# mdw771/beyond_dof

Hardware: AMD Instinct MI355X
Metric: multislice fwd+adjoint slice-steps/s (full Adam iteration: rotation, forward, loss, adjoint, gradient exchange, regulariser+Adam) (higher is better)
Workload: dtype f32

## Files before the change

### beyond_dof_amd/csrc/bdof_fft.h

```cpp
#pragma once
#include <hip/hip_runtime.h>

typedef float2 cf;

__device__ __forceinline__ cf cadd(cf a, cf b) { return make_float2(a.x + b.x, a.y + b.y); }
__device__ __forceinline__ cf csub(cf a, cf b) { return make_float2(a.x - b.x, a.y - b.y); }
__device__ __forceinline__ cf cmul(cf a, cf b) { return make_float2(a.x * b.x - a.y * b.y, a.x * b.y + a.y * b.x); }
__device__ __forceinline__ cf cmulc(cf a, cf b) { return make_float2(a.x * b.x + a.y * b.y, a.y * b.x - a.x * b.y); }
__device__ __forceinline__ cf cscale(cf a, float s) { return make_float2(a.x * s, a.y * s); }


template <int SIGN, bool EX> __device__ __forceinline__ cf tw_mul(cf u, cf w, cf wl) {
    if (SIGN > 0) { w.y = -w.y; wl.y = -wl.y; }
    if constexpr (EX) {
        const float lx = fmaf(u.x, wl.x, -(u.y * wl.y)), ly = fmaf(u.x, wl.y, u.y * wl.x);
        return make_float2(fmaf(u.x, w.x, fmaf(-u.y, w.y, lx)), fmaf(u.x, w.y, fmaf(u.y, w.x, ly)));
    } else return cmul(u, w);
}

template <int SIGN> __device__ __forceinline__ cf mul_si(cf a) {
    return SIGN > 0 ? make_float2(-a.y, a.x) : make_float2(a.y, -a.x);
}

template <int SIGN> __device__ __forceinline__ void dft2(cf& a, cf& b) {
    cf t = a;
    a = cadd(t, b);
    b = csub(t, b);
}

template <int SIGN> __device__ __forceinline__ void dft4(cf& a0, cf& a1, cf& a2, cf& a3) {
    cf s0 = cadd(a0, a2), s1 = csub(a0, a2), s2 = cadd(a1, a3), s3 = mul_si<SIGN>(csub(a1, a3));
    a0 = cadd(s0, s2);
    a2 = csub(s0, s2);
    a1 = cadd(s1, s3);
    a3 = csub(s1, s3);
}

template <int ROUND_> __device__ __forceinline__ float mul_sqrt_half(float t, const float* sq = nullptr) {
    if constexpr (ROUND_ != 0) {
        if (sq) return t * sq[ROUND_ - 1];
    }
    return fmaf(t, 0.70710678118654752f, t * 1.2101617e-8f);
}

template <int SIGN, int ROUND = 1>
__device__ __forceinline__ void dft8(cf& a0, cf& a1, cf& a2, cf& a3, cf& a4, cf& a5, cf& a6, cf& a7, const float* sq = nullptr) {
    dft4<SIGN>(a0, a2, a4, a6);
    dft4<SIGN>(a1, a3, a5, a7);
    const float s = (float)SIGN;
    cf o0 = a1;
    cf o1 = make_float2(mul_sqrt_half<ROUND>(a3.x - s * a3.y, sq), mul_sqrt_half<ROUND>(a3.y + s * a3.x, sq));
    cf o2 = mul_si<SIGN>(a5);
    cf o3 = make_float2(mul_sqrt_half<ROUND>(-a7.x - s * a7.y, sq), mul_sqrt_half<ROUND>(-a7.y + s * a7.x, sq));
    cf e0 = a0, e1 = a2, e2 = a4, e3 = a6;
    a0 = cadd(e0, o0); a4 = csub(e0, o0);
    a1 = cadd(e1, o1); a5 = csub(e1, o1);
    a2 = cadd(e2, o2); a6 = csub(e2, o2);
    a3 = cadd(e3, o3); a7 = csub(e3, o3);
}

template <int N> struct FftPlan;
template <> struct FftPlan<64>   { static constexpr int NS = 2, R0 = 8, R1 = 8, R2 = 1, R3 = 1; };
template <> struct FftPlan<128>  { static constexpr int NS = 3, R0 = 8, R1 = 2, R2 = 8, R3 = 1; };
template <> struct FftPlan<256>  { static constexpr int NS = 3, R0 = 8, R1 = 4, R2 = 8, R3 = 1; };
template <> struct FftPlan<512>  { static constexpr int NS = 3, R0 = 8, R1 = 8, R2 = 8, R3 = 1; };
template <> struct FftPlan<1024> { static constexpr int NS = 4, R0 = 8, R1 = 2, R2 = 8, R3 = 8; };

template <int N> struct FftTw {
    typedef FftPlan<N> P;
    static constexpr int RL = P::NS == 2 ? P::R1 : (P::NS == 3 ? P::R2 : P::R3);
    static constexpr int PL = N / RL;
    static constexpr int M1_R = P::NS > 2 ? P::R1 : 1, M1_P = P::R0;
    static constexpr int M2_R = P::NS > 3 ? P::R2 : 1, M2_P = P::R0 * P::R1;
    static constexpr int M1_OFF = 0, M1_CNT = P::NS > 2 ? M1_P * (M1_R - 1) : 0;
    static constexpr int M2_OFF = M1_CNT, M2_CNT = P::NS > 3 ? M2_P * (M2_R - 1) : 0;
    static constexpr int LDS_CNT = M1_CNT + M2_CNT > 0 ? M1_CNT + M2_CNT : 1;
    static constexpr int D1 = M1_R > 1 ? M1_R - 1 : 1, D2 = M2_R > 1 ? M2_R - 1 : 1;
    cf w[7];
    const cf* mid;
    const cf* tail;
    const float* sq = nullptr;

    template <bool LO = false>
    __device__ __forceinline__ void load(const cf* __restrict__ table, int tid, cf* lds_mid, cf* lds_tail) {
        constexpr int T = N / 8;
        for (int e = threadIdx.x; e < 7 * T; e += blockDim.x) {
            const int m = e / T + 1, j = e - (m - 1) * T;
            lds_tail[e] = table[m * j];
            if constexpr (LO) lds_tail[7 * T + e] = table[N + m * j];
        }
        for (int e = threadIdx.x; e < M1_CNT + M2_CNT; e += blockDim.x) {
            int k, m, step;
            if (e < M1_CNT) { k = e / D1; m = e % D1 + 1; step = N / (M1_P * M1_R); }
            else { const int f = e - M1_CNT; k = f / D2; m = f % D2 + 1; step = N / (M2_P * M2_R); }
            lds_mid[e] = table[m * k * step];
            if constexpr (LO) lds_mid[LDS_CNT + e] = table[N + m * k * step];
        }
        mid = lds_mid;
        tail = lds_tail;
        __syncthreads();
#pragma unroll
        for (int m = 1; m < 8; ++m) w[m - 1] = lds_tail[(m - 1) * T + tid];
    }
};

template <int R, int SIGN, int ROUND = 1> __device__ __forceinline__ void dftR(cf (&u)[8], int j, const float* sq = nullptr) {
    if constexpr (R == 8) dft8<SIGN, ROUND>(u[0], u[1], u[2], u[3], u[4], u[5], u[6], u[7], sq);
    else if constexpr (R == 4) {
        if (j == 0) dft4<SIGN>(u[0], u[1], u[2], u[3]); else dft4<SIGN>(u[4], u[5], u[6], u[7]);
    } else {
        if (j == 0) dft2<SIGN>(u[0], u[1]); else if (j == 1) dft2<SIGN>(u[2], u[3]);
        else if (j == 2) dft2<SIGN>(u[4], u[5]); else dft2<SIGN>(u[6], u[7]);
    }
}

template <int N, int R, class L> __device__ __forceinline__ void stage_read(cf (&u)[8], int tid, L& lds) {
    constexpr int T = N / 8, NB = 8 / R, TT = N / R;
#pragma unroll
    for (int j = 0; j < NB; ++j) {
        const int bs = lds.slot(tid + j * T);
#pragma unroll
        for (int m = 0; m < R; ++m) u[j * R + m] = lds.ld_at(bs, m * TT);
    }
}

template <int N, int SIGN, int R, int PP, int WHICH, int ROUND = 1, bool EX = false>
__device__ __forceinline__ void stage_compute(cf (&u)[8], const FftTw<N>& tw, int tid) {
    constexpr int T = N / 8, NB = 8 / R;
    typedef FftTw<N> TW;
#pragma unroll
    for (int j = 0; j < NB; ++j) {
        if constexpr (WHICH == 3) {
#pragma unroll
            for (int m = 1; m < R; ++m)
                u[j * R + m] = tw_mul<SIGN, EX>(u[j * R + m], tw.w[m - 1], EX ? tw.tail[(7 + m - 1) * T + tid] : tw.w[m - 1]);
        } else if constexpr (WHICH == 1 || WHICH == 2) {
            const int k = (tid + j * T) % PP;
            const cf* row = tw.mid + (WHICH == 1 ? TW::M1_OFF : TW::M2_OFF) + k * (R - 1);
#pragma unroll
            for (int m = 1; m < R; ++m) u[j * R + m] = tw_mul<SIGN, EX>(u[j * R + m], row[m - 1], row[(EX ? TW::LDS_CNT : 0) + m - 1]);
        }
        dftR<R, SIGN, EX ? 0 : ROUND>(u, j, tw.sq);
    }
}

template <int N, int R, int PP, class L> __device__ __forceinline__ void stage_write(const cf (&u)[8], int tid, L& lds) {
    constexpr int T = N / 8, NB = 8 / R;
#pragma unroll
    for (int j = 0; j < NB; ++j) {
        const int i = tid + j * T;
        const int k = i % PP;
        const int bs = lds.slot((i - k) * R + k);
#pragma unroll
        for (int q = 0; q < R; ++q) lds.st_at(bs, q * PP, u[j * R + q]);
    }
}

template <int N, int SIGN, int ROUND = 1, bool EX = false, class L>
__device__ __forceinline__ void line_fft(cf (&u)[8], const FftTw<N>& tw, int tid, L& lds) {
    typedef FftPlan<N> P;
    stage_compute<N, SIGN, P::R0, 1, 0, ROUND, EX>(u, tw, tid);
    lds.sync_r2w();
    stage_write<N, P::R0, 1>(u, tid, lds);
    lds.sync_w2r();
    stage_read<N, P::R1>(u, tid, lds);
    stage_compute<N, SIGN, P::R1, P::R0, (P::NS == 2 ? 3 : 1), ROUND, EX>(u, tw, tid);
    if constexpr (P::NS > 2) {
        lds.sync_r2w();
        stage_write<N, P::R1, P::R0>(u, tid, lds);
        lds.sync_w2r();
        stage_read<N, P::R2>(u, tid, lds);
        stage_compute<N, SIGN, P::R2, P::R0 * P::R1, (P::NS == 3 ? 3 : 2), ROUND, EX>(u, tw, tid);
    }
    if constexpr (P::NS > 3) {
        lds.sync_r2w();
        stage_write<N, P::R2, P::R0 * P::R1>(u, tid, lds);
        lds.sync_w2r();
        stage_read<N, P::R3>(u, tid, lds);
        stage_compute<N, SIGN, P::R3, P::R0 * P::R1 * P::R2, 3, ROUND, EX>(u, tw, tid);
    }
}

template <int N, int SIGN, int ROUND = 1, bool EX = false, class L>
__device__ __forceinline__ void line_fft_rest(cf (&u)[8], const FftTw<N>& tw, int tid, L& lds) {
    typedef FftPlan<N> P;
    stage_read<N, P::R1>(u, tid, lds);
    stage_compute<N, SIGN, P::R1, P::R0, (P::NS == 2 ? 3 : 1), ROUND, EX>(u, tw, tid);
    if constexpr (P::NS > 2) {
        lds.sync_r2w();
        stage_write<N, P::R1, P::R0>(u, tid, lds);
        lds.sync_w2r();
        stage_read<N, P::R2>(u, tid, lds);
        stage_compute<N, SIGN, P::R2, P::R0 * P::R1, (P::NS == 3 ? 3 : 2), ROUND, EX>(u, tw, tid);
    }
    if constexpr (P::NS > 3) {
        lds.sync_r2w();
        stage_write<N, P::R2, P::R0 * P::R1>(u, tid, lds);
        lds.sync_w2r();
        stage_read<N, P::R3>(u, tid, lds);
        stage_compute<N, SIGN, P::R3, P::R0 * P::R1 * P::R2, 3, ROUND, EX>(u, tw, tid);
    }
}

template <int N, int SIGN, int ROUND = 1, bool EX = false, class L>
__device__ __forceinline__ void line_fft_partial(cf (&u)[8], const FftTw<N>& tw, int tid, L& lds) {
    typedef FftPlan<N> P;
    stage_compute<N, SIGN, P::R0, 1, 0, ROUND, EX>(u, tw, tid);
    lds.sync_r2w();
    stage_write<N, P::R0, 1>(u, tid, lds);
    if constexpr (P::NS > 2) {
        lds.sync_w2r();
        stage_read<N, P::R1>(u, tid, lds);
        stage_compute<N, SIGN, P::R1, P::R0, 1, ROUND, EX>(u, tw, tid);
        lds.sync_r2w();
        stage_write<N, P::R1, P::R0>(u, tid, lds);
    }
    if constexpr (P::NS > 3) {
        lds.sync_w2r();
        stage_read<N, P::R2>(u, tid, lds);
        stage_compute<N, SIGN, P::R2, P::R0 * P::R1, 2, ROUND, EX>(u, tw, tid);
        lds.sync_r2w();
        stage_write<N, P::R2, P::R0 * P::R1>(u, tid, lds);
    }
}

template <int N, int SIGN, int ROUND = 1, bool EX = false, class L>
__device__ __forceinline__ void last_stage(cf (&u)[8], int j, L& lds, const cf* tail, const float* sq = nullptr) {
    constexpr int T = N / 8;
    cf w[7], wl[7];
#pragma unroll
    for (int m = 1; m < 8; ++m) {
        w[m - 1] = tail[(m - 1) * T + j];
        wl[m - 1] = tail[((EX ? 7 : 0) + m - 1) * T + j];
    }
    stage_read<N, 8>(u, j, lds);
#pragma unroll
    for (int m = 1; m < 8; ++m) u[m] = tw_mul<SIGN, EX>(u[m], w[m - 1], wl[m - 1]);
    dft8<SIGN, EX ? 0 : ROUND>(u[0], u[1], u[2], u[3], u[4], u[5], u[6], u[7], sq);
}
```

### beyond_dof_amd/csrc/bdof_kernels.h

```cpp
#pragma once
#include <type_traits>
#include "bdof_fft.h"

#define BDOF_THREADS 512

template <int N> struct RowCfg {
    static constexpr int T = N / 8;
    static constexpr int RPP = BDOF_THREADS / T;
    static constexpr int TILE = RPP > 16 ? RPP : 16;
    static constexpr int PASSES = TILE / RPP;
    static constexpr int NPAD = N + N / 16;
    static constexpr int RS = ((NPAD + 29) / 32) * 32 + 2;
    static constexpr int LDS_CF = TILE * RS;
    static constexpr int MIN_WAVES = N >= 1024 ? 2 : 4;
};

template <int T> struct RowLds {
    cf* base;
    __device__ __forceinline__ int slot(int i) const { return i + (i >> 4); }
    __device__ __forceinline__ cf ld_at(int base_slot, int c) const { return base[base_slot + c + (c >> 4)]; }
    __device__ __forceinline__ void st_at(int base_slot, int c, cf v) { base[base_slot + c + (c >> 4)] = v; }
    __device__ __forceinline__ void sync_w2r() { sync(); }
    __device__ __forceinline__ void sync_r2w() { sync(); }
    __device__ __forceinline__ void sync() {
// ... 646 lines not shown
    }
    if (a.meas) block_store_sum2(acc, acc2, a.partial + 2 * blockIdx.x);
}

#undef MEAS_OF
#undef WGT_OF

__global__ void k_sum_partials(const double* partial, int n, double scale, double* out) {
    double v = 0.0;
    for (int j = threadIdx.x; j < n; j += blockDim.x) v += partial[2 * j];
    __shared__ double wsum[4];
    v = wave_reduce_sum(v);
    if ((threadIdx.x & 63) == 0) wsum[threadIdx.x >> 6] = v;
    __syncthreads();
    if (threadIdx.x == 0) out[0] = (wsum[0] + wsum[1] + wsum[2] + wsum[3]) * scale;
}

struct RowBwdArgs {
    const cf* gin;
    const cf* tape;
    cf* gout;
    float2* grot;
    ObjView obj;
    int B, NX, z;
    float k;
    cf carrier;
    const cf* twiddle;
    const cf* pz;
    AdjCarrier ac;
    cf cshift;
    cf carrier_phi;
    float tape_scale;
    cf* gpsi0;
    int grot_S, grot_z;
    float sq[2];
};

template <int NY, int HIST, bool PF = false, bool GC = false, bool BIN = false>
__global__ __launch_bounds__(BDOF_THREADS, RowCfg<NY>::MIN_WAVES) void k_row_bwd(RowBwdArgs a) {
    typedef RowCfg<NY> C;
    __shared__ cf smem[C::LDS_CF];
    const int tid = threadIdx.x % C::T, rl = threadIdx.x / C::T;
    constexpr bool EX = false;
    __shared__ cf smem_tw[FftTw<NY>::LDS_CNT * (EX ? 2 : 1)];
    FftTw<NY> tw;
    __shared__ cf smem_tail[7 * C::T * (EX ? 2 : 1)];
    tw.template load<EX>(a.twiddle, tid, smem_tw, smem_tail);
    const float sq_bin[2] = {a.sq[0], a.sq[1]};
    tw.sq = BIN ? sq_bin : a.sq;
    const int ntiles = a.B * a.NX / C::TILE;
    for (int tile = blockIdx.x; tile < ntiles; tile += gridDim.x) {
        const int row0 = tile * C::TILE;
        const int b = row0 / a.NX, x0 = row0 - b * a.NX;
        const int y0 = a.obj.yoff ? a.obj.yoff[b] : 0;
        cf gam = make_float2(0.f, 0.f), t0 = make_float2(0.f, 0.f);
        if constexpr (GC) adj_carrier_load(a.ac, b, gam, t0);
        const int nbin = BIN ? a.obj.bin : 1;
#pragma nounroll
        for (int pass = 0; pass < C::PASSES; ++pass) {
            const int r = pass * C::RPP + rl;
            const int x = x0 + r;
            RowLds<C::T> lds{smem + r * C::RS};
            const size_t off = (size_t)(row0 + r) * NY;
            cf g[8], p[8];
            float2 db[8];
            if constexpr (BIN) load_obj_row_bin(a.obj, b, x, a.z, a.NX, y0, tid, C::T, db);
#pragma unroll
            for (int m = 0; m < 8; ++m) g[m] = a.gin[off + tid + m * C::T];
            const cf* psrc = HIST == 2 ? a.tape + (size_t)x * NY : a.tape + off;
#pragma unroll
            for (int m = 0; m < 8; ++m) p[m] = psrc[tid + m * C::T];
            if constexpr (!BIN) load_obj_row(a.obj, obj_src_row(a.obj, b, x, a.z, a.NX), y0, tid, C::T, db);
            cf pc[PF ? 8 : 1];
            if constexpr (PF) {
#pragma unroll
                for (int m = 0; m < 8; ++m) pc[m] = a.pz[(size_t)x * NY + tid + m * C::T];
            }
            if constexpr (HIST == 1 || HIST == 3) line_fft<NY, +1, 1, EX>(p, tw, tid, lds);
            if constexpr (HIST == 3) {
#pragma unroll
                for (int m = 0; m < 8; ++m) p[m] = cscale(p[m], a.tape_scale);
            }
            if constexpr (HIST == 1 || HIST == 2) {
#pragma unroll
                for (int m = 0; m < 8; ++m) p[m] = PF ? modulate_eps(p[m], pc[m], db[m]) : modulate_eps_s(p[m], a.carrier, db[m], a.cshift);
            }
            line_fft<NY, +1, 1, EX>(g, tw, tid, lds);
            float2* gdst = a.grot + (((size_t)b * a.grot_S + a.grot_z) * a.NX + x) * NY;
#pragma unroll
            for (int m = 0; m < 8; ++m) {
                const cf phi = cadd(p[m], PF ? pc[m] : a.carrier_phi);
                cf t = cmulc(g[m], phi);
                if constexpr (GC) t = cadd(cadd(t, cmulc(gam, p[m])), t0);
                const float2 gv = make_float2(a.k * t.y, -a.k * t.x);
                if constexpr (BIN) p[m] = gv;
                else gdst[tid + m * C::T] = gv;
                g[m] = cmulc(g[m], make_float2(1.f + db[m].x, db[m].y));
                if constexpr (GC) g[m] = cadd(g[m], cmulc(gam, csub(db[m], a.ac.cbm1)));
            }
            if constexpr (BIN) {
#pragma nounroll
                for (int j = 0; j < nbin; ++j, gdst += (size_t)a.NX * NY) {
#pragma unroll
                    for (int m = 0; m < 8; ++m) gdst[tid + m * C::T] = p[m];
                }
            }
            if (a.gpsi0) {
                cf* pd = a.gpsi0 + off;
#pragma unroll
                for (int m = 0; m < 8; ++m)
                    pd[tid + m * C::T] = GC ? cadd(g[m], cmulc(gam, make_float2(1.f + a.ac.cbm1.x, a.ac.cbm1.y))) : g[m];
            }
            if (a.gout) line_fft_partial<NY, -1, 1, EX>(g, tw, tid, lds);
        }
        if (a.gout) {
            __syncthreads();
            transposed_tail<NY, -1, 1, EX>(smem, a.gout + (size_t)b * NY * a.NX + x0, a.NX, 1.f, smem_tail, tw.sq);
            __syncthreads();
        }
    }
}

struct SliceArgs {
    const cf* in;
    const cf* probe;
    cf* out;
    cf* phi_out;
    ObjView obj;
    int B, R, z;
    cf carrier;
    cf cshift;
    const cf* tw_lead;
    const cf* tw_trail;
    const cf* h_lead;
    const cf* h_trail;
    float sq_lead[2], sq_trail[2];
};

template <int N, int SIGN, int ROUND = 1>
__device__ __forceinline__ void transposed_tail_mul(cf* smem, cf* __restrict__ dst, size_t ld, const cf* __restrict__ h, const cf* tail, const float* sq) {
    typedef RowCfg<N> C;
#pragma nounroll
    for (int pass = 0; pass < C::PASSES; ++pass) {
        const int q = threadIdx.x + pass * BDOF_THREADS;
        const int r = q % C::TILE, j = q / C::TILE;
        RowLds<C::T> lds{smem + r * C::RS};
        cf u[8], hv[8];
#pragma unroll
        for (int m = 0; m < 8; ++m) hv[m] = h[j + m * C::T];
        last_stage<N, SIGN, ROUND, false>(u, j, lds, tail, sq);
#pragma unroll
        for (int m = 0; m < 8; ++m) dst[(size_t)(j + m * C::T) * ld + r] = cmul(u[m], hv[m]);
    }
}

struct ObjRows {
    const int* look;
    long long plain0;
    int imax;
    int xmax;
    int mask;
};
__device__ __forceinline__ ObjRows obj_rows_of(const ObjView o, int b, int z, int NX) {
    ObjRows r;
    r.look = o.tab ? o.tab + ((long long)o.angle_of_b[b] * o.S + z) * o.volNX : (const int*)o.vol;
    r.plain0 = o.tab ? 0 : ((long long)b * o.S + z) * NX;
    r.imax = o.tab ? o.volNX - 1 : 0;
    r.xmax = o.tab ? o.volNX - 1 : 0x7fffffff;
    r.mask = o.tab ? -1 : 0;
    return r;
}
__device__ __forceinline__ int obj_rows_rel(const ObjRows r, int x) {
    const int s = r.look[(unsigned)min(x, r.imax)] & r.mask;
    return x <= r.xmax ? s + (x & ~r.mask) : -1;
}

template <int N> __device__ __forceinline__ void tw_fill(const cf* __restrict__ table, cf* lds_mid, cf* lds_tail) {
    typedef FftTw<N> TW;
    constexpr int T = N / 8;
    for (int e = threadIdx.x; e < 7 * T; e += blockDim.x) {
        const int m = e / T + 1, j = e - (m - 1) * T;
        lds_tail[e] = table[m * j];
    }
    for (int e = threadIdx.x; e < TW::M1_CNT + TW::M2_CNT; e += blockDim.x) {
        int k, m, step;
        if (e < TW::M1_CNT) { k = e / TW::D1; m = e % TW::D1 + 1; step = N / (TW::M1_P * TW::M1_R); }
        else { const int f = e - TW::M1_CNT; k = f / TW::D2; m = f % TW::D2 + 1; step = N / (TW::M2_P * TW::M2_R); }
        lds_mid[e] = table[m * k * step];
    }
}

template <int N> __device__ __forceinline__ void tw_select(FftTw<N>& tw, const cf* mid, const cf* tail, const float* sq, int tid) {
    asm volatile("" ::: "memory");
    tw.mid = mid;
    tw.tail = tail;
    tw.sq = sq;
#pragma unroll
    for (int m = 1; m < 8; ++m) tw.w[m - 1] = tail[(m - 1) * (N / 8) + tid];
}

template <int NY, bool FIRST, bool TAIL>
__global__ __launch_bounds__(BDOF_THREADS, RowCfg<NY>::MIN_WAVES) void k_slice_y(SliceArgs a) {
    typedef RowCfg<NY> C;
    __shared__ cf smem[C::LDS_CF];
    __shared__ cf smem_tw[2][FftTw<NY>::LDS_CNT];
    __shared__ cf smem_tail[2][7 * C::T];
    const int tid = threadIdx.x % C::T, rl = threadIdx.x / C::T;
    const float sql[2] = {a.sq_lead[0], a.sq_lead[1]}, sqt[2] = {a.sq_trail[0], a.sq_trail[1]};
    FftTw<NY> tw;
    if constexpr (!FIRST) tw_fill<NY>(a.tw_lead, smem_tw[0], smem_tail[0]);
    tw_fill<NY>(a.tw_trail, smem_tw[1], smem_tail[1]);
    __syncthreads();
    const int NX = a.R;
    const int ntiles = a.B * NX / C::TILE;
    for (int tile = blockIdx.x; tile < ntiles; tile += gridDim.x) {
        const int row0 = tile * C::TILE;
        const int b = row0 / NX, x0 = row0 - b * NX;
#pragma nounroll
        for (int pass = 0; pass < C::PASSES; ++pass) {
            const int r = pass * C::RPP + rl;
            const int x = x0 + r;
            RowLds<C::T> lds{smem + r * C::RS};
            cf u[8], hv[8];
            float2 db[8];
            const cf* src = FIRST ? a.probe + (size_t)x * NY : a.in + (size_t)(row0 + r) * NY;
#pragma unroll
            for (int m = 0; m < 8; ++m) u[m] = src[tid + m * C::T];
            load_obj_row(a.obj, obj_src_row(a.obj, b, x, a.z, NX), 0, tid, C::T, db);
            if constexpr (!FIRST) {
#pragma unroll
                for (int m = 0; m < 8; ++m) hv[m] = a.h_lead[tid + m * C::T];
                tw_select(tw, smem_tw[0], smem_tail[0], sql, tid);
                line_fft<NY, -1, 1, false>(u, tw, tid, lds);
#pragma unroll
                for (int m = 0; m < 8; ++m) u[m] = cmul(u[m], hv[m]);
                line_fft<NY, +1, 2, false>(u, tw, tid, lds);
            }
#pragma unroll
            for (int m = 0; m < 8; ++m) u[m] = modulate_eps_s(u[m], a.carrier, db[m], a.cshift);
            cf* pdst = a.phi_out + (size_t)(row0 + r) * NY;
#pragma unroll
            for (int m = 0; m < 8; ++m) pdst[tid + m * C::T] = u[m];
            tw_select(tw, smem_tw[1], smem_tail[1], sqt, tid);
            if constexpr (TAIL) {
                line_fft_partial<NY, -1, 1, false>(u, tw, tid, lds);
            } else {
#pragma unroll
                for (int m = 0; m < 8; ++m) hv[m] = a.h_trail[tid + m * C::T];
                line_fft<NY, -1, 1, false>(u, tw, tid, lds);
#pragma unroll
                for (int m = 0; m < 8; ++m) u[m] = cmul(u[m], hv[m]);
                line_fft_partial<NY, +1, 2, false>(u, tw, tid, lds);
            }
        }
        __syncthreads();
        cf* dst = a.out + (size_t)b * NY * NX + x0;
        if constexpr (TAIL) transposed_tail_mul<NY, -1, 1>(smem, dst, NX, a.h_trail, smem_tail[1], sqt);
        else transposed_tail<NY, +1, 2, false>(smem, dst, NX, 1.f, smem_tail[1], sqt);
        __syncthreads();
    }
}

template <int NX, bool BLK = false>
__global__ __launch_bounds__(BDOF_THREADS, RowCfg<NX>::MIN_WAVES) void k_slice_x(SliceArgs a) {
    typedef RowCfg<NX> C;
    typedef FftPlan<NX> P;
    __shared__ cf smem[C::LDS_CF];
    __shared__ cf smem_tw[2][FftTw<NX>::LDS_CNT];
    __shared__ cf smem_tail[2][7 * C::T];
    const int tid = threadIdx.x % C::T, rl = threadIdx.x / C::T;
    const float sql[2] = {a.sq_lead[0], a.sq_lead[1]}, sqt[2] = {a.sq_trail[0], a.sq_trail[1]};
    __shared__ int s_src[NX];
    FftTw<NX> tw;
    tw_fill<NX>(a.tw_lead, smem_tw[0], smem_tail[0]);
    tw_fill<NX>(a.tw_trail, smem_tw[1], smem_tail[1]);
    __syncthreads();
    const ObjView o = a.obj;
    const int NY = a.R;
    const int ntiles = a.B * NY / C::TILE;
    for (int tile = blockIdx.x; tile < ntiles; tile += gridDim.x) {
        const int row0 = tile * C::TILE;
        const int b = row0 / NY, y0 = row0 - b * NY;
        const ObjRows rows = obj_rows_of(o, b, a.z, NX);
        cf* const pdst = a.phi_out + (BLK ? (size_t)row0 * NX : (size_t)b * NX * NY);
        const int src_mine = (int)threadIdx.x < NX ? obj_rows_rel(rows, threadIdx.x) : -1;
#pragma nounroll
        for (int pass = 0; pass < C::PASSES; ++pass) {
            const int r = pass * C::RPP + rl;
            RowLds<C::T> lds{smem + r * C::RS};
            cf u[8], hv[8];
            const cf* src = a.in + (size_t)(row0 + r) * NX;
#pragma unroll
            for (int m = 0; m < 8; ++m) u[m] = src[tid + m * C::T];
#pragma unroll
            for (int m = 0; m < 8; ++m) hv[m] = a.h_lead[tid + m * C::T];
            tw_select(tw, smem_tw[0], smem_tail[0], sql, tid);
            line_fft<NX, -1, 1, false>(u, tw, tid, lds);
#pragma unroll
            for (int m = 0; m < 8; ++m) u[m] = cmul(u[m], hv[m]);
            line_fft_partial<NX, +1, 2, false>(u, tw, tid, lds);
        }
        if ((int)threadIdx.x < NX) s_src[threadIdx.x] = src_mine;
        __syncthreads();
        cf v[C::PASSES][8];
#pragma unroll
        for (int pass = 0; pass < C::PASSES; ++pass) {
            const int q = threadIdx.x + pass * BDOF_THREADS;
            const int r = q % C::TILE, j = q / C::TILE;
            RowLds<C::T> lds{smem + r * C::RS};
            const int yg = y0 + r, yc = min(max(yg, 0), o.volNY - 1);
            float2 db[8];
#pragma unroll
            for (int m = 0; m < 8; ++m) {
                const int srel = s_src[j + m * C::T];
                const float2 t = o.vol[(size_t)(rows.plain0 + max(srel, 0)) * o.volNY + yc];
                const bool in = srel >= 0 && yg == yc;
                db[m] = make_float2(in ? t.x : 0.f, in ? t.y : 0.f);
            }
            last_stage<NX, +1, 2, false>(v[pass], j, lds, smem_tail[0], sql);
#pragma unroll
            for (int m = 0; m < 8; ++m) {
                v[pass][m] = modulate_eps_s(v[pass][m], a.carrier, db[m], a.cshift);
                if constexpr (BLK) pdst[(unsigned)(q + m * C::T * C::TILE)] = v[pass][m];
                else pdst[(unsigned)((j + m * C::T) * NY + yg)] = v[pass][m];
            }
            tw.sq = sqt;
            stage_compute<NX, -1, P::R0, 1, 0, 1, false>(v[pass], tw, j);
        }
        __syncthreads();
#pragma unroll
        for (int pass = 0; pass < C::PASSES; ++pass) {
            const int q = threadIdx.x + pass * BDOF_THREADS;
            const int r = q % C::TILE, j = q / C::TILE;
            RowLds<C::T> lds{smem + r * C::RS};
            stage_write<NX, P::R0, 1>(v[pass], j, lds);
        }
        __syncthreads();
#pragma nounroll
        for (int pass = 0; pass < C::PASSES; ++pass) {
            const int r = pass * C::RPP + rl;
            RowLds<C::T> lds{smem + r * C::RS};
            cf u[8], hv[8];
#pragma unroll
            for (int m = 0; m < 8; ++m) hv[m] = a.h_trail[tid + m * C::T];
            tw_select(tw, smem_tw[1], smem_tail[1], sqt, tid);
            line_fft_rest<NX, -1, 1, false>(u, tw, tid, lds);
#pragma unroll
            for (int m = 0; m < 8; ++m) u[m] = cmul(u[m], hv[m]);
            line_fft_partial<NX, +1, 2, false>(u, tw, tid, lds);
        }
        __syncthreads();
        transposed_tail<NX, +1, 2, false>(smem, a.out + (size_t)b * NX * NY + y0, NY, 1.f, smem_tail[1], sqt);
        __syncthreads();
    }
}

struct SliceAdjArgs {
    const cf* in;
    const cf* phi;
    cf* out;
    float2* grot;
    ObjView obj;
    int B, R, z;
    float k;
    cf carrier_phi;
    const cf* tw_lead;
    const cf* tw_trail;
    const cf* h_lead;
    const cf* h_trail;
    float sq_lead[2], sq_trail[2];
};

template <int NY, bool HEAD, bool LAST>
__global__ __launch_bounds__(BDOF_THREADS, RowCfg<NY>::MIN_WAVES) void k_slice_y_adj(SliceAdjArgs a) {
    typedef RowCfg<NY> C;
    __shared__ cf smem[C::LDS_CF];
    __shared__ cf smem_tw[2][FftTw<NY>::LDS_CNT];
    __shared__ cf smem_tail[2][7 * C::T];
    const int tid = threadIdx.x % C::T, rl = threadIdx.x / C::T;
    const float sql[2] = {a.sq_lead[0], a.sq_lead[1]}, sqt[2] = {a.sq_trail[0], a.sq_trail[1]};
    FftTw<NY> tw;
    tw_fill<NY>(a.tw_lead, smem_tw[0], smem_tail[0]);
    if constexpr (!LAST) tw_fill<NY>(a.tw_trail, smem_tw[1], smem_tail[1]);
    __syncthreads();
    const int NX = a.R;
    const int ntiles = a.B * NX / C::TILE;
    for (int tile = blockIdx.x; tile < ntiles; tile += gridDim.x) {
        const int row0 = tile * C::TILE;
        const int b = row0 / NX, x0 = row0 - b * NX;
#pragma nounroll
        for (int pass = 0; pass < C::PASSES; ++pass) {
            const int r = pass * C::RPP + rl;
            const int x = x0 + r;
            RowLds<C::T> lds{smem + r * C::RS};
            const size_t off = (size_t)(row0 + r) * NY;
            cf g[8], p[8], hv[8];
            float2 db[8];
#pragma unroll
            for (int m = 0; m < 8; ++m) g[m] = a.in[off + tid + m * C::T];
            if constexpr (!HEAD) {
#pragma unroll
                for (int m = 0; m < 8; ++m) hv[m] = a.h_lead[tid + m * C::T];
            }
            auto load_phi_and_table = [&]() {
#pragma unroll
                for (int m = 0; m < 8; ++m) p[m] = a.phi[off + tid + m * C::T];
                load_obj_row(a.obj, obj_src_row(a.obj, b, x, a.z, NX), 0, tid, C::T, db);
            };
            tw_select(tw, smem_tw[0], smem_tail[0], sql, tid);
            if constexpr (HEAD) {
                load_phi_and_table();
                line_fft<NY, +1, 1, false>(g, tw, tid, lds);
            } else {
                line_fft<NY, -1, 1, false>(g, tw, tid, lds);
#pragma unroll
                for (int m = 0; m < 8; ++m) g[m] = cmulc(g[m], hv[m]);
                load_phi_and_table();
                line_fft<NY, +1, 2, false>(g, tw, tid, lds);
            }
            float2* gdst = a.grot + (((size_t)b * a.obj.S + a.z) * NX + x) * NY;
#pragma unroll
            for (int m = 0; m < 8; ++m) {
                const cf t = cmulc(g[m], cadd(p[m], a.carrier_phi));
                gdst[tid + m * C::T] = make_float2(a.k * t.y, -a.k * t.x);
                g[m] = cmulc(g[m], make_float2(1.f + db[m].x, db[m].y));
            }
            if constexpr (!LAST) {
#pragma unroll
                for (int m = 0; m < 8; ++m) hv[m] = a.h_trail[tid + m * C::T];
                tw_select(tw, smem_tw[1], smem_tail[1], sqt, tid);
                line_fft<NY, -1, 1, false>(g, tw, tid, lds);
#pragma unroll
                for (int m = 0; m < 8; ++m) g[m] = cmulc(g[m], hv[m]);
                line_fft_partial<NY, +1, 2, false>(g, tw, tid, lds);
            }
        }
        if constexpr (!LAST) {
            __syncthreads();
            transposed_tail<NY, +1, 2, false>(smem, a.out + (size_t)b * NY * NX + x0, NX, 1.f, smem_tail[1], sqt);
            __syncthreads();
        }
    }
}

template <int NX>
__global__ __launch_bounds__(BDOF_THREADS, RowCfg<NX>::MIN_WAVES) void k_slice_x_adj(SliceAdjArgs a) {
    typedef RowCfg<NX> C;
    typedef FftPlan<NX> P;
    __shared__ cf smem[C::LDS_CF];
    __shared__ cf smem_tw[2][FftTw<NX>::LDS_CNT];
    __shared__ cf smem_tail[2][7 * C::T];
    const int tid = threadIdx.x % C::T, rl = threadIdx.x / C::T;
    const float sql[2] = {a.sq_lead[0], a.sq_lead[1]}, sqt[2] = {a.sq_trail[0], a.sq_trail[1]};
    __shared__ int s_src[NX];
    FftTw<NX> tw;
    tw_fill<NX>(a.tw_lead, smem_tw[0], smem_tail[0]);
    tw_fill<NX>(a.tw_trail, smem_tw[1], smem_tail[1]);
    __syncthreads();
    const ObjView o = a.obj;
    const int NY = a.R;
    const int ntiles = a.B * NY / C::TILE;
    for (int tile = blockIdx.x; tile < ntiles; tile += gridDim.x) {
        const int row0 = tile * C::TILE;
        const int b = row0 / NY, y0 = row0 - b * NY;
        const ObjRows rows = obj_rows_of(o, b, a.z, NX);
        const cf* const psrc = a.phi + (size_t)row0 * NX;
        float2* const gdst = a.grot + ((size_t)b * o.S + a.z) * NX * NY;
        const int src_mine = (int)threadIdx.x < NX ? obj_rows_rel(rows, threadIdx.x) : -1;
#pragma nounroll
        for (int pass = 0; pass < C::PASSES; ++pass) {
            const int r = pass * C::RPP + rl;
            RowLds<C::T> lds{smem + r * C::RS};
            cf u[8], hv[8];
            const cf* src = a.in + (size_t)(row0 + r) * NX;
#pragma unroll
            for (int m = 0; m < 8; ++m) u[m] = src[tid + m * C::T];
#pragma unroll
            for (int m = 0; m < 8; ++m) hv[m] = a.h_lead[tid + m * C::T];
            tw_select(tw, smem_tw[0], smem_tail[0], sql, tid);
            line_fft<NX, -1, 1, false>(u, tw, tid, lds);
#pragma unroll
            for (int m = 0; m < 8; ++m) u[m] = cmulc(u[m], hv[m]);
            line_fft_partial<NX, +1, 2, false>(u, tw, tid, lds);
        }
        if ((int)threadIdx.x < NX) s_src[threadIdx.x] = src_mine;
        __syncthreads();
        cf v[C::PASSES][8];
#pragma unroll
        for (int pass = 0; pass < C::PASSES; ++pass) {
            const int q = threadIdx.x + pass * BDOF_THREADS;
            const int r = q % C::TILE, j = q / C::TILE;
            RowLds<C::T> lds{smem + r * C::RS};
            const int yg = y0 + r, yc = min(max(yg, 0), o.volNY - 1);
            float2 db[8];
            cf p[8];
#pragma unroll
            for (int m = 0; m < 8; ++m) {
                const int srel = s_src[j + m * C::T];
                const float2 t = o.vol[(size_t)(rows.plain0 + max(srel, 0)) * o.volNY + yc];
                const bool in = srel >= 0 && yg == yc;
                db[m] = make_float2(in ? t.x : 0.f, in ? t.y : 0.f);
            }
#pragma unroll
            for (int m = 0; m < 8; ++m) p[m] = psrc[(unsigned)(q + m * C::T * C::TILE)];
            last_stage<NX, +1, 2, false>(v[pass], j, lds, smem_tail[0], sql);
#pragma unroll
            for (int m = 0; m < 8; ++m) {
                const cf t = cmulc(v[pass][m], cadd(p[m], a.carrier_phi));
                gdst[(unsigned)((j + m * C::T) * NY + yg)] = make_float2(a.k * t.y, -a.k * t.x);
                v[pass][m] = cmulc(v[pass][m], make_float2(1.f + db[m].x, db[m].y));
            }
            tw.sq = sqt;
            stage_compute<NX, -1, P::R0, 1, 0, 1, false>(v[pass], tw, j);
        }
        __syncthreads();
#pragma unroll
        for (int pass = 0; pass < C::PASSES; ++pass) {
            const int q = threadIdx.x + pass * BDOF_THREADS;
            const int r = q % C::TILE, j = q / C::TILE;
            RowLds<C::T> lds{smem + r * C::RS};
            stage_write<NX, P::R0, 1>(v[pass], j, lds);
        }
        __syncthreads();
#pragma nounroll
        for (int pass = 0; pass < C::PASSES; ++pass) {
            const int r = pass * C::RPP + rl;
            RowLds<C::T> lds{smem + r * C::RS};
            cf u[8], hv[8];
#pragma unroll
            for (int m = 0; m < 8; ++m) hv[m] = a.h_trail[tid + m * C::T];
            tw_select(tw, smem_tw[1], smem_tail[1], sqt, tid);
            line_fft_rest<NX, -1, 1, false>(u, tw, tid, lds);
#pragma unroll
            for (int m = 0; m < 8; ++m) u[m] = cmulc(u[m], hv[m]);
            line_fft_partial<NX, +1, 2, false>(u, tw, tid, lds);
        }
        __syncthreads();
        transposed_tail<NX, +1, 2, false>(smem, a.out + (size_t)b * NX * NY + y0, NY, 1.f, smem_tail[1], sqt);
        __syncthreads();
    }
}

struct AdamArgs {
    const float2* x_old;
    float2* x_new;
    const float2* g;
    float2* m;
    float2* v;
    const float* mask;
    int NXv, NZv, NYv;
    float g_scale;
    float alpha_d, alpha_b, gamma;
    float lr, b1, b2, eps, inv_bc1, inv_bc2;
    float om_b1, om_b2;
    int clip;
    int x0, x1;
};

__device__ __forceinline__ float sgn(float v) { return (v > 0.f) - (v < 0.f); }

template <bool STORE_MV, class G>
__device__ __forceinline__ void adam_voxel(const AdamArgs& a, size_t idx, int x, int z, int y, G grad, float& nd, float& nb, float2& m, float2& v) {
    const float2 xv = a.x_old[idx];
    const float2 g = grad();
    float gd = g.x * a.g_scale + a.alpha_d * sgn(xv.x);
    float gb = g.y * a.g_scale + a.alpha_b * sgn(xv.y);
    if (a.gamma != 0.f) {
        const size_t sy = 1, sz = a.NYv, sx = (size_t)a.NZv * a.NYv;
        const float ym = a.x_old[idx - y * sy + ((y + a.NYv - 1) % a.NYv) * sy].x;
        const float yp = a.x_old[idx - y * sy + ((y + 1) % a.NYv) * sy].x;
        const float zm = a.x_old[idx - z * sz + ((z + a.NZv - 1) % a.NZv) * sz].x;
        const float zp = a.x_old[idx - z * sz + ((z + 1) % a.NZv) * sz].x;
        const float xm = a.x_old[idx - x * sx + ((x + a.NXv - 1) % a.NXv) * sx].x;
        const float xp = a.x_old[idx - x * sx + ((x + 1) % a.NXv) * sx].x;
        const float c = xv.x;
        gd += a.gamma * (sgn(c - ym) - sgn(yp - c) + sgn(c - zm) - sgn(zp - c) + sgn(c - xm) - sgn(xp - c));
    }
    m = a.m[idx];
    v = a.v[idx];
    m.x = a.om_b1 * gd + a.b1 * m.x;
    m.y = a.om_b1 * gb + a.b1 * m.y;
    v.x = a.om_b2 * gd * gd + a.b2 * v.x;
    v.y = a.om_b2 * gb * gb + a.b2 * v.y;
    if constexpr (STORE_MV) {
        a.m[idx] = m;
        a.v[idx] = v;
    }
    nd = xv.x - a.lr * (m.x * a.inv_bc1) / (sqrtf(v.x * a.inv_bc2) + a.eps);
    nb = xv.y - a.lr * (m.y * a.inv_bc1) / (sqrtf(v.y * a.inv_bc2) + a.eps);
    if (a.mask) { const float mk = a.mask[idx]; nd *= mk; nb *= mk; }
    if (a.clip) { nd = fmaxf(nd, 0.f); nb = fmaxf(nb, 0.f); }
}

struct RotAdjArgs {
    const float2* grot;
    float2* gvol;
    const int* off;
    const int* order;
    const int* angle_of_b;
    int B, n_src, n_dest, NY, accumulate;
    float scale;
    int* heavy_count;
    int* heavy_rows;
    int d0, d1;
};

#define BDOF_ROTADJ_MAXLIST 256

__device__ __forceinline__ void f4acc(float4& a, const float4 s) { a.x += s.x; a.y += s.y; a.z += s.z; a.w += s.w; }

template <bool FUSED> struct RotAdjK : RotAdjArgs {};
template <> struct RotAdjK<true> : RotAdjArgs {
    AdamArgs adam;
    float2* mod;
    double2* rowsum;
    float k;
};

__device__ __forceinline__ void rot_adjoint_tail(const RotAdjK<true>& a, int d, int v, float4 o, double& sx, double& sy) {
    const size_t idx = (size_t)d * a.NY + 2 * (size_t)v;
    const int x = d / a.adam.NZv, z = d % a.adam.NZv;
    if (a.gvol) reinterpret_cast<float4*>(a.gvol)[idx >> 1] = o;
    float2 n0, n1, m0, m1, v0, v1;
    adam_voxel<false>(a.adam, idx, x, z, 2 * v, [&] { return make_float2(o.x, o.y); }, n0.x, n0.y, m0, v0);
    adam_voxel<false>(a.adam, idx + 1, x, z, 2 * v + 1, [&] { return make_float2(o.z, o.w); }, n1.x, n1.y, m1, v1);
    reinterpret_cast<float4*>(a.adam.m)[idx >> 1] = make_float4(m0.x, m0.y, m1.x, m1.y);
    reinterpret_cast<float4*>(a.adam.v)[idx >> 1] = make_float4(v0.x, v0.y, v1.x, v1.y);
    reinterpret_cast<float4*>(a.adam.x_new)[idx >> 1] = make_float4(n0.x, n0.y, n1.x, n1.y);
    const float2 c0 = slice_modulation_m1(n0, a.k), c1 = slice_modulation_m1(n1, a.k);
    reinterpret_cast<float4*>(a.mod)[idx >> 1] = make_float4(c0.x, c0.y, c1.x, c1.y);
    sx += (double)c0.x;
    sy += (double)c0.y;
    sx += (double)c1.x;
    sy += (double)c1.y;
}

template <bool FUSED> __global__ __launch_bounds__(256) void k_rot_adjoint(RotAdjK<FUSED> a) {
    __shared__ int lists[4][BDOF_ROTADJ_MAXLIST];
    const int wave = threadIdx.x >> 6, lane = threadIdx.x & 63;
    int* list = lists[wave];
    const int nv = a.NY / 2;
    for (int d = a.d0 + blockIdx.x * 4 + wave; d < a.d1; d += gridDim.x * 4) {
        int total = 0;
        for (int b0 = 0; b0 < a.B; b0 += 64) {
            const int b = b0 + lane;
            int e0 = 0, cnt = 0;
            const int* order = a.order;
            if (b < a.B) {
                const int ang = a.angle_of_b[b];
                const int* off = a.off + (size_t)ang * (a.n_dest + 1);
                e0 = off[d];
                cnt = off[d + 1] - e0;
                order = a.order + (size_t)ang * a.n_src;
            }
            int incl = cnt;
#pragma unroll
            for (int o = 1; o < 64; o <<= 1) {
                const int t = __shfl_up(incl, o, 64);
                if (lane >= o) incl += t;
            }
            const int chunk_total = __shfl(incl, 63, 64);
            if (total + chunk_total <= BDOF_ROTADJ_MAXLIST) {
                int pos = total + incl - cnt;
                for (int e = 0; e < cnt; ++e) list[pos++] = b * a.n_src + order[e0 + e];
            }
            total += chunk_total;
        }
        __builtin_amdgcn_fence(__ATOMIC_RELEASE, "wavefront");
        __builtin_amdgcn_wave_barrier();
        __builtin_amdgcn_fence(__ATOMIC_ACQUIRE, "wavefront");
        if (total > BDOF_ROTADJ_MAXLIST) {
            if (lane == 0) a.heavy_rows[atomicAdd(a.heavy_count, 1)] = d;
            continue;
        }
        float4* drow = reinterpret_cast<float4*>(a.gvol + (size_t)d * a.NY);
        double sx = 0.0, sy = 0.0;
        for (int v0 = 0; v0 < nv; v0 += 256) {
            float4 acc[4];
            bool ok[4];
#pragma unroll
            for (int c = 0; c < 4; ++c) { acc[c] = make_float4(0.f, 0.f, 0.f, 0.f); ok[c] = v0 + c * 64 + lane < nv; }
            int e = 0;
            for (; e + 2 <= total; e += 2) {
                const float4* r0 = reinterpret_cast<const float4*>(a.grot + (size_t)list[e] * a.NY) + v0 + lane;
                const float4* r1 = reinterpret_cast<const float4*>(a.grot + (size_t)list[e + 1] * a.NY) + v0 + lane;
                float4 s0[4], s1[4];
#pragma unroll
                for (int c = 0; c < 4; ++c) if (ok[c]) { s0[c] = r0[c * 64]; s1[c] = r1[c * 64]; }
#pragma unroll
                for (int c = 0; c < 4; ++c) if (ok[c]) { f4acc(acc[c], s0[c]); f4acc(acc[c], s1[c]); }
            }
            for (; e < total; ++e) {
                const float4* r0 = reinterpret_cast<const float4*>(a.grot + (size_t)list[e] * a.NY) + v0 + lane;
#pragma unroll
                for (int c = 0; c < 4; ++c) if (ok[c]) f4acc(acc[c], r0[c * 64]);
            }
#pragma unroll
            for (int c = 0; c < 4; ++c) {
                if (!ok[c]) continue;
                float4 o = make_float4(acc[c].x * a.scale, acc[c].y * a.scale, acc[c].z * a.scale, acc[c].w * a.scale);
                if constexpr (FUSED) {
                    rot_adjoint_tail(a, d, v0 + c * 64 + lane, o, sx, sy);
                } else {
                    float4* dst = drow + v0 + c * 64 + lane;
                    if (a.accumulate) f4acc(o, *dst);
                    *dst = o;
                }
            }
        }
        if constexpr (FUSED) {
            if (a.rowsum) {
                sx = wave_reduce_sum(sx);
                sy = wave_reduce_sum(sy);
                if (lane == 0) a.rowsum[d] = make_double2(sx, sy);
            }
        }
        __builtin_amdgcn_fence(__ATOMIC_RELEASE, "wavefront");
        __builtin_amdgcn_wave_barrier();
        __builtin_amdgcn_fence(__ATOMIC_ACQUIRE, "wavefront");
    }
}

template <bool FUSED> __global__ __launch_bounds__(256) void k_rot_adjoint_heavy(RotAdjK<FUSED> a) {
    __shared__ int stage[256];
    const int nheavy = *a.heavy_count;
    const int nv = a.NY / 2;
    for (int i = blockIdx.x; i < nheavy; i += gridDim.x) {
        const int d = a.heavy_rows[i];
        double sx = 0.0, sy = 0.0;
        for (int v0 = 0; v0 < nv; v0 += 256) {
            const int v = v0 + threadIdx.x;
            float4 acc = make_float4(0.f, 0.f, 0.f, 0.f);
            for (int b = 0; b < a.B; ++b) {
                const int ang = a.angle_of_b[b];
                const int* off = a.off + (size_t)ang * (a.n_dest + 1);
                const int* order = a.order + (size_t)ang * a.n_src;
                const int e0 = off[d], e1 = off[d + 1];
                for (int c0 = e0; c0 < e1; c0 += 256) {
                    const int n = min(256, e1 - c0);
                    __syncthreads();
                    if ((int)threadIdx.x < n) stage[threadIdx.x] = b * a.n_src + order[c0 + threadIdx.x];
                    __syncthreads();
                    if (v < nv) {
                        int e = 0;
                        for (; e + 4 <= n; e += 4) {
                            const float4 s0 = reinterpret_cast<const float4*>(a.grot + (size_t)stage[e] * a.NY)[v];
                            const float4 s1 = reinterpret_cast<const float4*>(a.grot + (size_t)stage[e + 1] * a.NY)[v];
                            const float4 s2 = reinterpret_cast<const float4*>(a.grot + (size_t)stage[e + 2] * a.NY)[v];
                            const float4 s3 = reinterpret_cast<const float4*>(a.grot + (size_t)stage[e + 3] * a.NY)[v];
                            f4acc(acc, s0); f4acc(acc, s1); f4acc(acc, s2); f4acc(acc, s3);
                        }
                        for (; e < n; ++e) f4acc(acc, reinterpret_cast<const float4*>(a.grot + (size_t)stage[e] * a.NY)[v]);
                    }
                }
            }
            if (v < nv) {
                float4* dst = reinterpret_cast<float4*>(a.gvol + (size_t)d * a.NY) + v;
                float4 o = make_float4(acc.x * a.scale, acc.y * a.scale, acc.z * a.scale, acc.w * a.scale);
                if constexpr (FUSED) {
                    rot_adjoint_tail(a, d, v, o, sx, sy);
                } else {
                    if (a.accumulate) f4acc(o, *dst);
                    *dst = o;
                }
            }
        }
        if constexpr (FUSED) {
            if (a.rowsum) {
                if (block_sum2<256>(sx, sy)) a.rowsum[d] = make_double2(sx, sy);
                __syncthreads();
            }
        }
    }
}

__global__ __launch_bounds__(256) void k_adam(AdamArgs a) {
    const size_t slab = (size_t)a.NZv * a.NYv;
    const size_t first = (size_t)a.x0 * slab, total = (size_t)(a.x1 - a.x0) * slab;
    const size_t per_xcd = (total + 7) / 8;
    const size_t lane0 = (size_t)(blockIdx.x >> 3) * blockDim.x + threadIdx.x, stride = (size_t)(gridDim.x >> 3) * blockDim.x;
    const size_t c0 = (size_t)(blockIdx.x & 7) * per_xcd, c1 = c0 + per_xcd < total ? c0 + per_xcd : total;
    for (size_t loc = c0 + lane0; loc < c1; loc += stride) {
        const size_t idx = first + loc;
        const int y = idx % a.NYv;
        const size_t r = idx / a.NYv;
        const int z = r % a.NZv;
        const int x = r / a.NZv;
        float nd, nb;
        float2 m, v;
        adam_voxel<true>(a, idx, x, z, y, [&] { return a.g[idx]; }, nd, nb, m, v);
        a.x_new[idx] = make_float2(nd, nb);
    }
}

#define BDOF_TILE_MAXLIST 1024
struct TileGradArgs {
    const float2* grot;
    float2* gvol;
    const int* tab;
    const int* x0;
    const int* y0;
    int B, TX, TY, volNX, volNY, z0, nz, accumulate;
};
__global__ __launch_bounds__(256) void k_tiles_grad_add(TileGradArgs a) {
    __shared__ int lb[BDOF_TILE_MAXLIST];
    __shared__ int nlist, resume;
    for (int xg = blockIdx.x; xg < a.volNX; xg += gridDim.x) {
        for (int b_next = 0; b_next < a.B;) {
            __syncthreads();
            if (threadIdx.x == 0) {
                int n = 0, b = b_next;
                for (; b < a.B; ++b) {
                    const int x = xg - a.x0[b];
                    if (x < 0 || x >= a.TX) continue;
                    if (n == BDOF_TILE_MAXLIST) break;
                    lb[n++] = b;
                }
                nlist = n;
                resume = b;
            }
            __syncthreads();
            const int n = nlist;
            b_next = resume;
            for (int yg = threadIdx.x; yg < a.volNY; yg += blockDim.x) {
// ... 674 lines not shown
```

Before: 232,700.

## Write first FFT stage in place to drop barrier and per-pass register arrays

The fused column-pass kernels now write each pass's first-stage FFT results back to the same LDS slots they were read from. A matching strided read is added at the start of the remaining stages. This removes a __syncthreads between computing and writing, and removes the need to hold PASSES×8 complex values in registers, which should lower register pressure and improve occupancy. The trade-off is a different LDS access pattern for the write and the next read, which may cause bank conflicts, and the change relies on the in-place index mapping being correct.

```diff
diff --git a/beyond_dof_amd/csrc/bdof_fft.h b/beyond_dof_amd/csrc/bdof_fft.h
--- a/beyond_dof_amd/csrc/bdof_fft.h
+++ b/beyond_dof_amd/csrc/bdof_fft.h
@@ -181,10 +181,28 @@
     }
 }
 
+template <int N, class L> __device__ __forceinline__ void stage_write_inplace(const cf (&u)[8], int j, L& lds) {
+    constexpr int T = N / 8;
+    const int bs = lds.slot(j);
+#pragma unroll
+    for (int q = 0; q < 8; ++q) lds.st_at(bs, q * T, u[q]);
+}
+
+template <int N, int R, class L> __device__ __forceinline__ void stage_read_inplace(cf (&u)[8], int tid, L& lds) {
+    constexpr int T = N / 8, NB = 8 / R, TT = N / R;
+    static_assert(T % 8 == 0 && TT % 8 == 0, "in-place first stage: lines of at least 64 points");
+    const int bs = lds.slot(tid / 8 + T * (tid % 8));
+#pragma unroll
+    for (int j = 0; j < NB; ++j) {
+#pragma unroll
+        for (int m = 0; m < R; ++m) u[j * R + m] = lds.ld_at(bs, (j * T + m * TT) / 8);
+    }
+}
+
 template <int N, int SIGN, int ROUND = 1, bool EX = false, class L>
 __device__ __forceinline__ void line_fft_rest(cf (&u)[8], const FftTw<N>& tw, int tid, L& lds) {
     typedef FftPlan<N> P;
-    stage_read<N, P::R1>(u, tid, lds);
+    stage_read_inplace<N, P::R1>(u, tid, lds);
     stage_compute<N, SIGN, P::R1, P::R0, (P::NS == 2 ? 3 : 1), ROUND, EX>(u, tw, tid);
     if constexpr (P::NS > 2) {
         lds.sync_r2w();
diff --git a/beyond_dof_amd/csrc/bdof_kernels.h b/beyond_dof_amd/csrc/bdof_kernels.h
--- a/beyond_dof_amd/csrc/bdof_kernels.h
+++ b/beyond_dof_amd/csrc/bdof_kernels.h
@@ -972,7 +972,6 @@
         }
         if ((int)threadIdx.x < NX) s_src[threadIdx.x] = src_mine;
         __syncthreads();
-        cf v[C::PASSES][8];
 #pragma unroll
         for (int pass = 0; pass < C::PASSES; ++pass) {
             const int q = threadIdx.x + pass * BDOF_THREADS;
@@ -980,6 +979,7 @@
             RowLds<C::T> lds{smem + r * C::RS};
             const int yg = y0 + r, yc = min(max(yg, 0), o.volNY - 1);
             float2 db[8];
+            cf v[8];
 #pragma unroll
             for (int m = 0; m < 8; ++m) {
                 const int srel = s_src[j + m * C::T];
@@ -987,23 +987,16 @@
                 const bool in = srel >= 0 && yg == yc;
                 db[m] = make_float2(in ? t.x : 0.f, in ? t.y : 0.f);
             }
-            last_stage<NX, +1, 2, false>(v[pass], j, lds, smem_tail[0], sql);
+            last_stage<NX, +1, 2, false>(v, j, lds, smem_tail[0], sql);
 #pragma unroll
             for (int m = 0; m < 8; ++m) {
-                v[pass][m] = modulate_eps_s(v[pass][m], a.carrier, db[m], a.cshift);
-                if constexpr (BLK) pdst[(unsigned)(q + m * C::T * C::TILE)] = v[pass][m];
-                else pdst[(unsigned)((j + m * C::T) * NY + yg)] = v[pass][m];
+                v[m] = modulate_eps_s(v[m], a.carrier, db[m], a.cshift);
+                if constexpr (BLK) pdst[(unsigned)(q + m * C::T * C::TILE)] = v[m];
+                else pdst[(unsigned)((j + m * C::T) * NY + yg)] = v[m];
             }
             tw.sq = sqt;
-            stage_compute<NX, -1, P::R0, 1, 0, 1, false>(v[pass], tw, j);
-        }
-        __syncthreads();
-#pragma unroll
-        for (int pass = 0; pass < C::PASSES; ++pass) {
-            const int q = threadIdx.x + pass * BDOF_THREADS;
-            const int r = q % C::TILE, j = q / C::TILE;
-            RowLds<C::T> lds{smem + r * C::RS};
-            stage_write<NX, P::R0, 1>(v[pass], j, lds);
+            stage_compute<NX, -1, P::R0, 1, 0, 1, false>(v, tw, j);
+            stage_write_inplace<NX>(v, j, lds);
         }
         __syncthreads();
 #pragma nounroll
@@ -1155,7 +1148,6 @@
         }
         if ((int)threadIdx.x < NX) s_src[threadIdx.x] = src_mine;
         __syncthreads();
-        cf v[C::PASSES][8];
 #pragma unroll
         for (int pass = 0; pass < C::PASSES; ++pass) {
             const int q = threadIdx.x + pass * BDOF_THREADS;
@@ -1163,7 +1155,7 @@
             RowLds<C::T> lds{smem + r * C::RS};
             const int yg = y0 + r, yc = min(max(yg, 0), o.volNY - 1);
             float2 db[8];
-            cf p[8];
+            cf p[8], v[8];
 #pragma unroll
             for (int m = 0; m < 8; ++m) {
                 const int srel = s_src[j + m * C::T];
@@ -1173,23 +1165,16 @@
             }
 #pragma unroll
             for (int m = 0; m < 8; ++m) p[m] = psrc[(unsigned)(q + m * C::T * C::TILE)];
-            last_stage<NX, +1, 2, false>(v[pass], j, lds, smem_tail[0], sql);
+            last_stage<NX, +1, 2, false>(v, j, lds, smem_tail[0], sql);
 #pragma unroll
             for (int m = 0; m < 8; ++m) {
-                const cf t = cmulc(v[pass][m], cadd(p[m], a.carrier_phi));
+                const cf t = cmulc(v[m], cadd(p[m], a.carrier_phi));
                 gdst[(unsigned)((j + m * C::T) * NY + yg)] = make_float2(a.k * t.y, -a.k * t.x);
-                v[pass][m] = cmulc(v[pass][m], make_float2(1.f + db[m].x, db[m].y));
+                v[m] = cmulc(v[m], make_float2(1.f + db[m].x, db[m].y));
             }
             tw.sq = sqt;
-            stage_compute<NX, -1, P::R0, 1, 0, 1, false>(v[pass], tw, j);
-        }
-        __syncthreads();
-#pragma unroll
-        for (int pass = 0; pass < C::PASSES; ++pass) {
-            const int q = threadIdx.x + pass * BDOF_THREADS;
-            const int r = q % C::TILE, j = q / C::TILE;
-            RowLds<C::T> lds{smem + r * C::RS};
-            stage_write<NX, P::R0, 1>(v[pass], j, lds);
+            stage_compute<NX, -1, P::R0, 1, 0, 1, false>(v, tw, j);
+            stage_write_inplace<NX>(v, j, lds);
         }
         __syncthreads();
 #pragma nounroll
```

Result: no change. 233,200, median of 5 (+0.2%).
